# NoelShin/zutis

Measured on AMD Instinct MI355X. Metric: images/sec, COCO2017-val-shaped ViT-B/16 dense semantic segmentation @336px (ZUTIS forward + semantic predict), batches of 32 per GPU, 3 independent batches in flight, higher is better.
Workload: dtype f16x3 (fp32-class)

## Files before the change

### zutis_amd/csrc/attention.hip

```cpp
#include "common.h"
#include <type_traits>

struct AttnArgs {
  const half_t* Q; long ldq, sQ;
  const half_t* K; long ldk, sK;
  const half_t* V; long ldv, sV;
  half_t* O; long ldo, sO;
  int Tq, Tk, H, nqb, groups;
  float scale_log2;
  int causal;
  long planeQ, planeK, planeV, planeO;
  int ksplit, kchunk;
  float* part_o; float* part_m; float* part_l;
};

typedef __fp16 fp16x4 __attribute__((__vector_size__(4 * sizeof(__fp16))));
typedef __attribute__((address_space(3))) fp16x4* lds_fp16x4_ptr;

#define KT 64
#define VS 96

#define ZH_ATTN_LAZY_LOG2 8.0f

__device__ __forceinline__ float zh_xor32_max(float x) {
  float a = x, b = x;
  asm volatile("s_nop 1\n\tv_permlane32_swap_b32 %0, %1" : "+v"(a), "+v"(b));
  float r;
  asm("v_max_f32 %0, %1, %2" : "=v"(r) : "v"(a), "v"(b));
  return r;
}
__device__ __forceinline__ float zh_xor32_sum(float x) {
  float a = x, b = x;
  asm volatile("s_nop 1\n\tv_permlane32_swap_b32 %0, %1" : "+v"(a), "+v"(b));
  return a + b;
}

template <int DH, int NWAVE, int X3, int PIPE>
__global__ __launch_bounds__(64 * NWAVE, X3 ? 2 : (DH == 64 ? 3 : 2)) void attn_f16_kernel(AttnArgs p) {
  static_assert(!PIPE || X3, "the pipelined loop exists for the split-pair kernels");
  constexpr int NT = 64 * NWAVE;
  constexpr int KS = DH + 8;
  constexpr int NKS = DH / 16;
  constexpr int NDT = DH / 32;
  constexpr int CPR = DH / 8;
  constexpr int KTT = X3 ? 32 : KT;
  constexpr int NU = KTT / 32;
  constexpr int NLD = (KTT * CPR + NT - 1) / NT;
  constexpr bool LDFULL = (KTT * CPR) % NT == 0;
  __shared__ __attribute__((aligned(16))) half_t sKb[2][KTT * KS];
  __shared__ __attribute__((aligned(16))) half_t sKl[X3 ? 2 : 1][X3 ? KTT * KS : 8];
  __shared__ __attribute__((aligned(16))) half_t sVb[2][KTT * VS];
  __shared__ __attribute__((aligned(16))) half_t sVl[X3 ? 2 : 1][X3 ? KTT * VS : 8];

  const int tid = threadIdx.x, lane = tid & 63, wave = tid >> 6;
  const int id = blockIdx.y * gridDim.x + blockIdx.x;
  const int per_group = p.nqb * p.ksplit;
  const int item = (id & 7) * (int)(gridDim.x >> 3) + (id >> 3);
  if (item >= p.groups * per_group) return;
  const int group = item / per_group;
  const int qbs = item - group * per_group;
  const int qb = qbs / p.ksplit, ks = qbs - qb * p.ksplit;
  const int head = group % p.H, img = group / p.H;
  const int q0 = qb * (32 * NWAVE) + wave * 32;
  const int ql = lane & 31, hh = lane >> 5;
  const long hoff = (long)head * DH;

  const int key0 = ks * p.kchunk;
  const int key_end = p.ksplit > 1 ? min(p.Tk, key0 + p.kchunk) : p.Tk;
  const half_t* Q = p.Q + (long)img * p.sQ + hoff;
  const half_t* K = p.K + (long)img * p.sK + hoff;
  const half_t* V = p.V + (long)img * p.sV + hoff;

  half8_t qf[NKS], qfl[X3 ? NKS : 1];
  const half_t* qp = Q + (long)min(q0 + ql, p.Tq - 1) * p.ldq + 8 * hh;
#pragma unroll
  for (int ks = 0; ks < NKS; ++ks) qf[ks] = *(const half8_t*)(qp + 16 * ks);
  if (X3) {
#pragma unroll
    for (int ks = 0; ks < NKS; ++ks) qfl[ks] = *(const half8_t*)(qp + p.planeQ + 16 * ks);
  }

  f32x16 oacc[NDT];
#pragma unroll
  for (int d = 0; d < NDT; ++d)
#pragma unroll
    for (int r = 0; r < 16; ++r) oacc[d][r] = 0.f;
  float m_run = -INFINITY;
  f32x16 lacc;
#pragma unroll
  for (int r = 0; r < 16; ++r) lacc[r] = 0.f;
  float l_run = 0.f;
  half8_t ones;
#pragma unroll
  for (int i = 0; i < 8; ++i) ones[i] = (half_t)1.0f;

  struct TileRegs { half8_t k[NLD], v[NLD], kl[X3 ? NLD : 1], vl[X3 ? NLD : 1]; };
  TileRegs ra;
  const unsigned ldk2 = (unsigned)p.ldk * 2u, ldv2 = (unsigned)p.ldv * 2u;
  const char* const Kl = (const char*)(K + p.planeK);
  const char* const Vl = (const char*)(V + p.planeV);
  auto load_k = [&](int kbase, TileRegs& r) {
#pragma unroll
    for (int i = 0; i < NLD; ++i) {
      const int c = tid + i * NT;
      const int row = c / CPR, cc = c - row * CPR;
      if (LDFULL || c < KTT * CPR) {
        const unsigned ok = (unsigned)min(kbase + row, key_end - 1) * ldk2 + (unsigned)cc * 16u;
        r.k[i] = *(const half8_t*)((const char*)K + ok);
        if (X3) r.kl[i] = *(const half8_t*)(Kl + ok);
      }
    }
  };
  auto load_v = [&](int kbase, TileRegs& r) {
#pragma unroll
    for (int i = 0; i < NLD; ++i) {
      const int c = tid + i * NT;
      const int row = c / CPR, cc = c - row * CPR;
      if (LDFULL || c < KTT * CPR) {
        const unsigned ov = (unsigned)min(kbase + row, key_end - 1) * ldv2 + (unsigned)cc * 16u;
        r.v[i] = *(const half8_t*)((const char*)V + ov);
        if (X3) r.vl[i] = *(const half8_t*)(Vl + ov);
      }
    }
  };
  auto store_k = [&](int buf, const TileRegs& r) {
#pragma unroll
    for (int i = 0; i < NLD; ++i) {
      const int c = tid + i * NT;
      const int row = c / CPR, cc = c - row * CPR;
      if (LDFULL || c < KTT * CPR) {
        *(half8_t*)(sKb[buf] + row * KS + cc * 8) = r.k[i];
        if (X3) *(half8_t*)(sKl[buf] + row * KS + cc * 8) = r.kl[i];
      }
    }
  };
  auto store_v = [&](int buf, const TileRegs& r) {
#pragma unroll
    for (int i = 0; i < NLD; ++i) {
      const int c = tid + i * NT;
      const int row = c / CPR, cc = c - row * CPR;
      if (LDFULL || c < KTT * CPR) {
        *(half8_t*)(sVb[buf] + row * VS + cc * 8) = r.v[i];
        if (X3) *(half8_t*)(sVl[buf] + row * VS + cc * 8) = r.vl[i];
      }
    }
  };

  const int krow = (ql & 0x13) | ((ql & 4) << 1) | ((ql & 8) >> 1);
  const int tr_row = 8 * hh + ((lane & 15) >> 2);
  const int tr_col = 16 * ((lane >> 4) & 1) + 4 * (lane & 3);

  int ntiles = (max(key_end - key0, 0) + KTT - 1) / KTT;
  if (p.causal) {
    const int qlast = min(p.Tq, (qb + 1) * (32 * NWAVE)) - 1;
    ntiles = min(ntiles, qlast / KTT + 1);
  }
  const int qidx = q0 + ql;
  const bool active = q0 < p.Tq;

  auto qk = [&](int t, f32x16 (&s)[NU]) {
    const half_t* sK = sKb[t & 1];
#pragma unroll
    for (int u = 0; u < NU; ++u) {
#pragma unroll
      for (int r = 0; r < 16; ++r) s[u][r] = 0.f;
      const half_t* kp = sK + (32 * u + krow) * KS + 8 * hh;
#pragma unroll
      for (int ks = 0; ks < NKS; ++ks) {
        half8_t kf = *(const half8_t*)(kp + 16 * ks);
        half8_t kl;
        if (X3) kl = *(const half8_t*)(sKl[t & 1] + (32 * u + krow) * KS + 8 * hh + 16 * ks);
        s[u] = __builtin_amdgcn_mfma_f32_32x32x16_f16(kf, qf[ks], s[u], 0, 0, 0);
        if (X3) {
          s[u] = __builtin_amdgcn_mfma_f32_32x32x16_f16(kl, qf[ks], s[u], 0, 0, 0);
          s[u] = __builtin_amdgcn_mfma_f32_32x32x16_f16(kf, qfl[ks], s[u], 0, 0, 0);
        }
      }
    }
  };
  typedef unsigned u32x4 __attribute__((ext_vector_type(4)));
  struct PFrag { u32x4 hi[NU][2], lo[X3 ? NU : 1][2]; };
  auto softmax = [&](int t, f32x16 (&s)[NU], PFrag& P, auto masked) {
    constexpr bool MASKED = decltype(masked)::value;
    const int kbase = key0 + t * KTT;
    float mx = -INFINITY;
    if (MASKED && (kbase + KTT > key_end || (p.causal && kbase + KTT - 1 > q0))) {
#pragma unroll
      for (int u = 0; u < NU; ++u)
#pragma unroll
        for (int r = 0; r < 16; ++r) {
          const int key = kbase + 32 * u + 16 * (r >> 3) + 8 * hh + (r & 7);
          if (key >= key_end || (p.causal && key > qidx)) s[u][r] = -INFINITY;
        }
    }
    {
      float m4[4] = {mx, mx, mx, mx};
#pragma unroll
      for (int u = 0; u < NU; ++u)
#pragma unroll
        for (int r = 0; r < 16; r += 8) {
          m4[0] = fmaxf(fmaxf(m4[0], s[u][r + 0]), s[u][r + 1]);
          m4[1] = fmaxf(fmaxf(m4[1], s[u][r + 2]), s[u][r + 3]);
          m4[2] = fmaxf(fmaxf(m4[2], s[u][r + 4]), s[u][r + 5]);
          m4[3] = fmaxf(fmaxf(m4[3], s[u][r + 6]), s[u][r + 7]);
        }
      mx = fmaxf(fmaxf(m4[0], m4[1]), fmaxf(m4[2], m4[3]));
    }
    mx = zh_xor32_max(mx);
    const float m_cand = mx * p.scale_log2;
    const float m_new = m_cand > m_run + ZH_ATTN_LAZY_LOG2 ? m_cand : m_run;
    const float alpha = __builtin_amdgcn_exp2f(m_run - m_new);
    m_run = m_new;
    float lsum2[2] = {0.f, 0.f};
#pragma unroll
    for (int u = 0; u < NU; ++u)
#pragma unroll
      for (int r = 0; r < 16; r += 2) {
        const float e0 = __builtin_amdgcn_exp2f(__builtin_fmaf(s[u][r], p.scale_log2, -m_new));
        const float e1 = __builtin_amdgcn_exp2f(__builtin_fmaf(s[u][r + 1], p.scale_log2, -m_new));
        if (X3) { lsum2[0] += e0; lsum2[1] += e1; }
        const half2_t eh2 = {(half_t)e0, (half_t)e1};
        unsigned eh = __builtin_bit_cast(unsigned, eh2);
        if (X3) {
          unsigned el;
          asm("v_fma_mixlo_f16 %0, -%1, 1.0, %2 op_sel:[0,0,0] op_sel_hi:[1,0,0]\n\t"
              "v_fma_mixhi_f16 %0, -%1, 1.0, %3 op_sel:[1,0,0] op_sel_hi:[1,0,0]"
              : "=&v"(el) : "v"(eh), "v"(e0), "v"(e1));
          P.lo[u][r >> 3][(r >> 1) & 3] = el;
        }
        P.hi[u][r >> 3][(r >> 1) & 3] = eh;
      }
    if (__any(alpha != 1.0f)) {
#pragma unroll
      for (int d = 0; d < NDT; ++d)
#pragma unroll
        for (int r = 0; r < 16; ++r) oacc[d][r] *= alpha;
      if (!X3) {
#pragma unroll
        for (int r = 0; r < 16; ++r) lacc[r] *= alpha;
      }
    }
    if (X3) l_run = l_run * alpha + (lsum2[0] + lsum2[1]);
  };
  auto pv = [&](int t, const PFrag& P) {
    const half_t* sV = sVb[t & 1];
#pragma unroll
    for (int u = 0; u < NU; ++u)
#pragma unroll
      for (int ks = 0; ks < 2; ++ks) {
        if (!X3) lacc = __builtin_amdgcn_mfma_f32_32x32x16_f16(ones, __builtin_bit_cast(half8_t, P.hi[u][ks]), lacc, 0, 0, 0);
        const half_t* vp = sV + (32 * u + 16 * ks + tr_row) * VS + tr_col;
#pragma unroll
        for (int d = 0; d < NDT; ++d) {
          fp16x4 lo = __builtin_amdgcn_ds_read_tr16_b64_v4f16((lds_fp16x4_ptr)(vp + 32 * d));
          fp16x4 hi = __builtin_amdgcn_ds_read_tr16_b64_v4f16((lds_fp16x4_ptr)(vp + 32 * d + 4 * VS));
          half8_t vf;
          __builtin_memcpy(&vf, &lo, 8);
          __builtin_memcpy(((char*)&vf) + 8, &hi, 8);
          half8_t vl;
          if (X3) {
            const half_t* vq = sVl[t & 1] + (32 * u + 16 * ks + tr_row) * VS + tr_col;
            fp16x4 llo = __builtin_amdgcn_ds_read_tr16_b64_v4f16((lds_fp16x4_ptr)(vq + 32 * d));
            fp16x4 lhi = __builtin_amdgcn_ds_read_tr16_b64_v4f16((lds_fp16x4_ptr)(vq + 32 * d + 4 * VS));
            __builtin_memcpy(&vl, &llo, 8);
            __builtin_memcpy(((char*)&vl) + 8, &lhi, 8);
          }
          const half8_t pf = __builtin_bit_cast(half8_t, P.hi[u][ks]);
          oacc[d] = __builtin_amdgcn_mfma_f32_32x32x16_f16(vf, pf, oacc[d], 0, 0, 0);
          if (X3) {
            oacc[d] = __builtin_amdgcn_mfma_f32_32x32x16_f16(vl, pf, oacc[d], 0, 0, 0);
            oacc[d] = __builtin_amdgcn_mfma_f32_32x32x16_f16(vf, __builtin_bit_cast(half8_t, P.lo[u][ks]), oacc[d], 0, 0, 0);
          }
        }
      }
  };

  if (PIPE && !p.causal) {
    load_k(key0, ra);
    load_v(key0, ra);
    store_k(0, ra);
    store_v(0, ra);
    if (ntiles > 1) { load_k(key0 + KTT, ra); store_k(1, ra); }
    __syncthreads();
    f32x16 sA[NU], sB[NU];
    PFrag P;
    if (active) qk(0, sA);
    __syncthreads();
    auto step = [&](int t, auto par, f32x16 (&cur)[NU], f32x16 (&nxt)[NU]) {
      constexpr int PAR = decltype(par)::value;
      if (t + 2 < ntiles) load_k(key0 + (t + 2) * KTT, ra);
      load_v(key0 + (t + 1) * KTT, ra);
      if (active) {
        qk(PAR ^ 1, nxt);
        softmax(t, cur, P, std::false_type{});
        pv(PAR, P);
      }
      if (t + 2 < ntiles) store_k(PAR, ra);
      store_v(PAR ^ 1, ra);
      __syncthreads();
    };
    int t = 0;
    for (; t + 2 < ntiles; t += 2) {
      step(t, std::integral_constant<int, 0>{}, sA, sB);
      step(t + 1, std::integral_constant<int, 1>{}, sB, sA);
    }
    if (t + 1 < ntiles) {
      step(t, std::integral_constant<int, 0>{}, sA, sB);
      if (active) { softmax(t + 1, sB, P, std::true_type{}); pv(1, P); }
    } else if (active) {
      softmax(t, sA, P, std::true_type{});
      pv(0, P);
    }
  } else {
  auto load_tile = [&](int kbase, TileRegs& r) { load_k(kbase, r); load_v(kbase, r); };
  auto store_tile = [&](int buf, const TileRegs& r) { store_k(buf, r); store_v(buf, r); };
  load_tile(key0, ra);
  store_tile(0, ra);
  __syncthreads();
  auto compute = [&](int t) {
    if (active) {
      f32x16 s[NU];
      PFrag P;
      qk(t, s);
      softmax(t, s, P, std::true_type{});
      pv(t, P);
    }
  };

  for (int t = 0; t < ntiles; t += 2) {
    if (t + 1 < ntiles) load_tile(key0 + (t + 1) * KTT, ra);
    compute(t);
    if (t + 1 < ntiles) store_tile(1, ra);
    __syncthreads();
    if (t + 1 >= ntiles) break;
    if (t + 2 < ntiles) load_tile(key0 + (t + 2) * KTT, ra);
    compute(t + 1);
    if (t + 2 < ntiles) store_tile(0, ra);
    __syncthreads();
  }
  }

  for (int once = 0; once < 1; ++once) {
  const float l_row = X3 ? zh_xor32_sum(l_run) : lacc[0];
  const int qr = q0 + ql;
  if (p.ksplit > 1) {
    if (qr < p.Tq) {
      float* po = p.part_o + (((long)ks * (p.groups / p.H) + img) * p.Tq + qr) * ((long)p.H * DH) + hoff + 4 * hh;
#pragma unroll
      for (int d = 0; d < NDT; ++d)
#pragma unroll
        for (int g = 0; g < 4; ++g)
          *(f32x4*)(po + 32 * d + 8 * g) = (f32x4){oacc[d][4 * g], oacc[d][4 * g + 1], oacc[d][4 * g + 2], oacc[d][4 * g + 3]};
      if (hh == 0) {
        const long mi = ((long)ks * p.groups + group) * p.Tq + qr;
        p.part_m[mi] = m_run;
        p.part_l[mi] = l_row;
      }
    }
    continue;
  }
  const float inv = 1.0f / l_row;
  if (qr < p.Tq) {
    half_t* op = p.O + (long)img * p.sO + (long)qr * p.ldo + hoff + 4 * hh;
#pragma unroll
    for (int d = 0; d < NDT; ++d)
#pragma unroll
      for (int g = 0; g < 4; ++g) {
        const f32x4 o = {oacc[d][4 * g] * inv, oacc[d][4 * g + 1] * inv, oacc[d][4 * g + 2] * inv, oacc[d][4 * g + 3] * inv};
        zh_store_h4(op + 32 * d + 8 * g, p.planeO, o);
      }
  }
  }
}

__global__ __launch_bounds__(256) void attn_combine_kernel(const float* part_o, const float* part_m, const float* part_l, half_t* O, long ldo, long sO,
                                                           long planeO, int S, int B, int H, int Tq, int DH) {
  const int D = H * DH, c4 = D / 4;
  const long i = (long)blockIdx.x * 256 + threadIdx.x;
  if (i >= (long)B * Tq * c4) return;
  const int col = (int)(i % c4) * 4;
  const long row = i / c4;
  const int img = (int)(row / Tq), q = (int)(row - (long)img * Tq), head = col / DH;
  float m = -INFINITY;
  for (int s = 0; s < S; ++s) m = fmaxf(m, part_m[(((long)s * B + img) * H + head) * Tq + q]);
  f32x4 acc = {0.f, 0.f, 0.f, 0.f};
  float l = 0.f;
  for (int s = 0; s < S; ++s) {
    const long mi = (((long)s * B + img) * H + head) * Tq + q;
    const float w = __builtin_amdgcn_exp2f(part_m[mi] - m);
    l += w * part_l[mi];
    acc += *(const f32x4*)(part_o + (((long)s * B + img) * Tq + q) * D + col) * w;
  }
  const float inv = 1.0f / l;
  zh_store_h4(O + (long)img * sO + (long)q * ldo + col, planeO, acc * inv);
}

static int attention_launch(const void* Q, long ldq, long strideQ, const void* K, long ldk, long strideK,
                            const void* V, long ldv, long strideV, void* O, long ldo, long strideO,
                            int batch, int heads, int Tq, int Tk, int head_dim, float scale, int causal,
                            long planeQ, long planeK, long planeV, long planeO, hipStream_t stream, int ksplit = 1, void* workspace = nullptr,
                            size_t workspace_bytes = 0) {
  ZH_CHECK_ARG(Q && K && V && O, "zh_attention_f16: null operand");
  ZH_CHECK_ARG(batch > 0 && heads > 0 && Tq > 0 && Tk > 0, "zh_attention_f16: bad shape");
  ZH_CHECK_ARG(head_dim == 64 || head_dim == 96, "zh_attention_f16: head_dim %d not in {64, 96}", head_dim);
  ZH_CHECK_ARG(ldq % 8 == 0 && ldk % 8 == 0 && ldv % 8 == 0 && ldo % 4 == 0 && strideQ % 8 == 0 && strideK % 8 == 0 &&
                   strideV % 8 == 0 && strideO % 4 == 0 && planeQ % 8 == 0 && planeK % 8 == 0 && planeV % 8 == 0 && planeO % 4 == 0,
               "zh_attention_f16: row/batch/plane strides must keep 16-byte (Q,K,V) / 8-byte (O) alignment");
  ZH_CHECK_ARG(((uintptr_t)Q & 15) == 0 && ((uintptr_t)K & 15) == 0 && ((uintptr_t)V & 15) == 0 && ((uintptr_t)O & 7) == 0,
               "zh_attention_f16: misaligned pointer");
  ZH_CHECK_ARG(heads < 65536 && batch < 65536, "zh_attention_f16: heads/batch exceed grid limits");
  ZH_CHECK_ARG((long)Tk * ldk * 2 < (1L << 32) && (long)Tk * ldv * 2 < (1L << 32), "zh_attention_f16: Tk * ldk (ldv) exceeds 2^31 elements");
  ZH_CHECK_ARG((planeQ != 0) == (planeK != 0) && (planeQ != 0) == (planeV != 0),
               "zh_attention_f16: the split-pair mode needs the lo planes of Q, K and V (all three or none)");
  AttnArgs p;
  p.Q = (const half_t*)Q; p.ldq = ldq; p.sQ = strideQ;
  p.K = (const half_t*)K; p.ldk = ldk; p.sK = strideK;
  p.V = (const half_t*)V; p.ldv = ldv; p.sV = strideV;
  p.O = (half_t*)O; p.ldo = ldo; p.sO = strideO;
  p.Tq = Tq; p.Tk = Tk; p.H = heads;
  p.scale_log2 = scale * 1.4426950408889634f;
  p.causal = causal;
  p.planeQ = planeQ; p.planeK = planeK; p.planeV = planeV; p.planeO = planeO;
  const bool x3 = planeQ != 0;
  p.nqb = zh_cdiv(Tq, 128);
  p.groups = heads * batch;
  p.ksplit = 1; p.kchunk = 0; p.part_o = p.part_m = p.part_l = nullptr;
  if (ksplit > 1) {
    ZH_CHECK_ARG(!causal && ksplit <= 64, "zh_attention_f16_splitk: ksplit %d not in 1..64 (and not for the causal form)", ksplit);
    const int ktt = x3 ? 32 : 64;
    p.ksplit = ksplit;
    p.kchunk = zh_cdiv(zh_cdiv(Tk, ktt), ksplit) * ktt;
    ZH_CHECK_ARG((long)(ksplit - 1) * p.kchunk < Tk, "zh_attention_f16_splitk: ksplit %d leaves an empty key chunk for Tk = %d", ksplit, Tk);
    const size_t no = (size_t)ksplit * batch * Tq * heads * head_dim, nm = (size_t)ksplit * batch * heads * Tq;
    ZH_CHECK_ARG(workspace && workspace_bytes >= (no + 2 * nm) * 4 && ((uintptr_t)workspace & 15) == 0,
                 "zh_attention_f16_splitk: workspace too small or misaligned (%zu < %zu)", workspace_bytes, (no + 2 * nm) * 4);
    p.part_o = (float*)workspace; p.part_m = p.part_o + no; p.part_l = p.part_m + nm;
  }
  const long items = (long)p.groups * p.nqb * p.ksplit;
  ZH_CHECK_ARG(items < (1L << 31) - 8, "zh_attention_f16: grid too large");
  const long nblk = (long)zh_cdiv(items, 8) * 8;
  ZH_CHECK_ARG(nblk < (1L << 31), "zh_attention_f16: grid too large");
  dim3 grid((unsigned)nblk);
  const bool pipe = x3 && (head_dim == 96 || zh_cdiv(nblk, 512L) <= zh_cdiv(nblk, 768L));
  if (head_dim == 64) {
    if (x3 && pipe) hipLaunchKernelGGL((attn_f16_kernel<64, 4, 1, 1>), grid, dim3(256), 0, stream, p);
    else if (x3) hipLaunchKernelGGL((attn_f16_kernel<64, 4, 1, 0>), grid, dim3(256), 0, stream, p);
    else hipLaunchKernelGGL((attn_f16_kernel<64, 4, 0, 0>), grid, dim3(256), 0, stream, p);
  } else {
    if (x3 && pipe) hipLaunchKernelGGL((attn_f16_kernel<96, 4, 1, 1>), grid, dim3(256), 0, stream, p);
    else if (x3) hipLaunchKernelGGL((attn_f16_kernel<96, 4, 1, 0>), grid, dim3(256), 0, stream, p);
    else hipLaunchKernelGGL((attn_f16_kernel<96, 4, 0, 0>), grid, dim3(256), 0, stream, p);
  }
  ZH_CHECK_LAUNCH("zh_attention_f16");
  if (p.ksplit > 1) {
    const long n4 = (long)batch * Tq * heads * head_dim / 4;
    hipLaunchKernelGGL(attn_combine_kernel, dim3((unsigned)zh_cdiv(n4, 256)), dim3(256), 0, stream, p.part_o, p.part_m, p.part_l, p.O, ldo, strideO,
                       planeO, p.ksplit, batch, heads, Tq, head_dim);
    ZH_CHECK_LAUNCH("zh_attention_f16_splitk (combine)");
  }
  return ZH_OK;
}

extern "C" size_t zh_attention_splitk_workspace_size(int batch, int heads, int Tq, int head_dim, int ksplit) {
  return ((size_t)ksplit * batch * Tq * heads * head_dim + 2 * (size_t)ksplit * batch * heads * Tq) * 4;
}
extern "C" int zh_attention_f16_splitk(const void* Q, long ldq, long strideQ, const void* K, long ldk, long strideK,
                                       const void* V, long ldv, long strideV, void* O, long ldo, long strideO,
                                       int batch, int heads, int Tq, int Tk, int head_dim, float scale,
                                       long planeQ, long planeK, long planeV, long planeO, int ksplit, void* workspace, size_t workspace_bytes,
                                       hipStream_t stream) {
  return attention_launch(Q, ldq, strideQ, K, ldk, strideK, V, ldv, strideV, O, ldo, strideO, batch, heads, Tq, Tk, head_dim,
                          scale, 0, planeQ, planeK, planeV, planeO, stream, ksplit, workspace, workspace_bytes);
}

extern "C" int zh_attention_f16(const void* Q, long ldq, long strideQ, const void* K, long ldk, long strideK,
                                const void* V, long ldv, long strideV, void* O, long ldo, long strideO,
                                int batch, int heads, int Tq, int Tk, int head_dim, float scale,
                                long planeQ, long planeK, long planeV, long planeO, hipStream_t stream) {
  return attention_launch(Q, ldq, strideQ, K, ldk, strideK, V, ldv, strideV, O, ldo, strideO, batch, heads, Tq, Tk, head_dim,
                          scale, 0, planeQ, planeK, planeV, planeO, stream);
}

extern "C" int zh_attention_causal_f16(const void* Q, long ldq, long strideQ, const void* K, long ldk, long strideK,
                                       const void* V, long ldv, long strideV, void* O, long ldo, long strideO,
                                       int batch, int heads, int T, int head_dim, float scale,
                                       long planeQ, long planeK, long planeV, long planeO, hipStream_t stream) {
  return attention_launch(Q, ldq, strideQ, K, ldk, strideK, V, ldv, strideV, O, ldo, strideO, batch, heads, T, T, head_dim,
                          scale, 1, planeQ, planeK, planeV, planeO, stream);
}
```

Before: 3073.

## Stream K/V tiles into LDS via direct global-to-LDS DMA with 3-stage ring

For the split-pair (X3) attention kernels, K and V tiles are now loaded straight from global memory into LDS with global_load_lds_dwordx4 instead of going through registers and ds_write. A three-stage ring buffer with vmcnt-based partial waits replaces the old register double-buffering. The LDS layout becomes unpadded and XOR-swizzled, and the qk and pv read addressing is changed to match. This is meant to free VGPRs and the issue slots spent on LDS stores, and to hide more load latency. The cost is extra LDS per block, reliance on hand-written inline asm for m0 and waitcnt, and tricky counter bookkeeping that can cause races if it is wrong.

```diff
diff --git a/zutis_amd/csrc/attention.hip b/zutis_amd/csrc/attention.hip
--- a/zutis_amd/csrc/attention.hip
+++ b/zutis_amd/csrc/attention.hip
@@ -18,7 +18,6 @@
 typedef __attribute__((address_space(3))) fp16x4* lds_fp16x4_ptr;
 
 #define KT 64
-#define VS 96
 
 #define ZH_ATTN_LAZY_LOG2 8.0f
 
@@ -35,22 +34,49 @@
   return a + b;
 }
 
+__device__ __forceinline__ void attn_dma16(unsigned lds, unsigned off, const char* base) {
+  asm volatile("s_nop 2\n\ts_mov_b32 m0, %0\n\ts_nop 0\n\tglobal_load_lds_dwordx4 %1, %2" :: "s"(lds), "v"(off), "s"(base) : "memory");
+}
+__device__ __forceinline__ const char* attn_sgpr_ptr(const void* ptr) {
+  const uintptr_t v = (uintptr_t)ptr;
+  return (const char*)(((uintptr_t)(unsigned)__builtin_amdgcn_readfirstlane((int)(v >> 32)) << 32) |
+                       (uintptr_t)(unsigned)__builtin_amdgcn_readfirstlane((int)(unsigned)v));
+}
+template <int NP, int MAXC>
+__device__ __forceinline__ void attn_wait_barrier(int c) {
+  static_assert(MAXC * NP < 64, "vmcnt is a 6-bit counter");
+  if constexpr (MAXC > 0) {
+    if (c >= MAXC) {
+      asm volatile("s_waitcnt vmcnt(%0) lgkmcnt(0)\n\ts_barrier" :: "n"(MAXC * NP) : "memory");
+      return;
+    }
+    attn_wait_barrier<NP, MAXC - 1>(c);
+  } else {
+    asm volatile("s_waitcnt vmcnt(0) lgkmcnt(0)\n\ts_barrier" ::: "memory");
+  }
+}
+
 template <int DH, int NWAVE, int X3, int PIPE>
 __global__ __launch_bounds__(64 * NWAVE, X3 ? 2 : (DH == 64 ? 3 : 2)) void attn_f16_kernel(AttnArgs p) {
   static_assert(!PIPE || X3, "the pipelined loop exists for the split-pair kernels");
-  constexpr int NT = 64 * NWAVE;
-  constexpr int KS = DH + 8;
   constexpr int NKS = DH / 16;
   constexpr int NDT = DH / 32;
   constexpr int CPR = DH / 8;
   constexpr int KTT = X3 ? 32 : KT;
   constexpr int NU = KTT / 32;
+  constexpr int PLANE = KTT * DH;
+  constexpr int STAGE = 4 * PLANE;
+  constexpr int NST = 3;
+  constexpr int PPP = PLANE / 512;
+  constexpr int NPW = 2 * PPP / NWAVE;
+  static_assert(!X3 || 2 * PPP % NWAVE == 0, "whole pieces per wave");
+  constexpr int KS = DH + 8, VS = 96;
+  constexpr int NT = 64 * NWAVE;
   constexpr int NLD = (KTT * CPR + NT - 1) / NT;
   constexpr bool LDFULL = (KTT * CPR) % NT == 0;
-  __shared__ __attribute__((aligned(16))) half_t sKb[2][KTT * KS];
-  __shared__ __attribute__((aligned(16))) half_t sKl[X3 ? 2 : 1][X3 ? KTT * KS : 8];
-  __shared__ __attribute__((aligned(16))) half_t sVb[2][KTT * VS];
-  __shared__ __attribute__((aligned(16))) half_t sVl[X3 ? 2 : 1][X3 ? KTT * VS : 8];
+  __shared__ __attribute__((aligned(16))) half_t smem[X3 ? NST * STAGE : 2 * KTT * (KS + VS)];
+  auto k_at = [&](int st) { return smem + (X3 ? st * STAGE : st * KTT * KS); };
+  auto v_at = [&](int st) { return smem + (X3 ? st * STAGE + 2 * PLANE : 2 * KTT * KS + st * KTT * VS); };
 
   const int tid = threadIdx.x, lane = tid & 63, wave = tid >> 6;
   const int id = blockIdx.y * gridDim.x + blockIdx.x;
@@ -71,85 +97,6 @@
   const half_t* K = p.K + (long)img * p.sK + hoff;
   const half_t* V = p.V + (long)img * p.sV + hoff;
 
-  half8_t qf[NKS], qfl[X3 ? NKS : 1];
-  const half_t* qp = Q + (long)min(q0 + ql, p.Tq - 1) * p.ldq + 8 * hh;
-#pragma unroll
-  for (int ks = 0; ks < NKS; ++ks) qf[ks] = *(const half8_t*)(qp + 16 * ks);
-  if (X3) {
-#pragma unroll
-    for (int ks = 0; ks < NKS; ++ks) qfl[ks] = *(const half8_t*)(qp + p.planeQ + 16 * ks);
-  }
-
-  f32x16 oacc[NDT];
-#pragma unroll
-  for (int d = 0; d < NDT; ++d)
-#pragma unroll
-    for (int r = 0; r < 16; ++r) oacc[d][r] = 0.f;
-  float m_run = -INFINITY;
-  f32x16 lacc;
-#pragma unroll
-  for (int r = 0; r < 16; ++r) lacc[r] = 0.f;
-  float l_run = 0.f;
-  half8_t ones;
-#pragma unroll
-  for (int i = 0; i < 8; ++i) ones[i] = (half_t)1.0f;
-
-  struct TileRegs { half8_t k[NLD], v[NLD], kl[X3 ? NLD : 1], vl[X3 ? NLD : 1]; };
-  TileRegs ra;
-  const unsigned ldk2 = (unsigned)p.ldk * 2u, ldv2 = (unsigned)p.ldv * 2u;
-  const char* const Kl = (const char*)(K + p.planeK);
-  const char* const Vl = (const char*)(V + p.planeV);
-  auto load_k = [&](int kbase, TileRegs& r) {
-#pragma unroll
-    for (int i = 0; i < NLD; ++i) {
-      const int c = tid + i * NT;
-      const int row = c / CPR, cc = c - row * CPR;
-      if (LDFULL || c < KTT * CPR) {
-        const unsigned ok = (unsigned)min(kbase + row, key_end - 1) * ldk2 + (unsigned)cc * 16u;
-        r.k[i] = *(const half8_t*)((const char*)K + ok);
-        if (X3) r.kl[i] = *(const half8_t*)(Kl + ok);
-      }
-    }
-  };
-  auto load_v = [&](int kbase, TileRegs& r) {
-#pragma unroll
-    for (int i = 0; i < NLD; ++i) {
-      const int c = tid + i * NT;
-      const int row = c / CPR, cc = c - row * CPR;
-      if (LDFULL || c < KTT * CPR) {
-        const unsigned ov = (unsigned)min(kbase + row, key_end - 1) * ldv2 + (unsigned)cc * 16u;
-        r.v[i] = *(const half8_t*)((const char*)V + ov);
-        if (X3) r.vl[i] = *(const half8_t*)(Vl + ov);
-      }
-    }
-  };
-  auto store_k = [&](int buf, const TileRegs& r) {
-#pragma unroll
-    for (int i = 0; i < NLD; ++i) {
-      const int c = tid + i * NT;
-      const int row = c / CPR, cc = c - row * CPR;
-      if (LDFULL || c < KTT * CPR) {
-        *(half8_t*)(sKb[buf] + row * KS + cc * 8) = r.k[i];
-        if (X3) *(half8_t*)(sKl[buf] + row * KS + cc * 8) = r.kl[i];
-      }
-    }
-  };
-  auto store_v = [&](int buf, const TileRegs& r) {
-#pragma unroll
-    for (int i = 0; i < NLD; ++i) {
-      const int c = tid + i * NT;
-      const int row = c / CPR, cc = c - row * CPR;
-      if (LDFULL || c < KTT * CPR) {
-        *(half8_t*)(sVb[buf] + row * VS + cc * 8) = r.v[i];
-        if (X3) *(half8_t*)(sVl[buf] + row * VS + cc * 8) = r.vl[i];
-      }
-    }
-  };
-
-  const int krow = (ql & 0x13) | ((ql & 4) << 1) | ((ql & 8) >> 1);
-  const int tr_row = 8 * hh + ((lane & 15) >> 2);
-  const int tr_col = 16 * ((lane >> 4) & 1) + 4 * (lane & 3);
-
   int ntiles = (max(key_end - key0, 0) + KTT - 1) / KTT;
   if (p.causal) {
     const int qlast = min(p.Tq, (qb + 1) * (32 * NWAVE)) - 1;
@@ -158,18 +105,126 @@
   const int qidx = q0 + ql;
   const bool active = q0 < p.Tq;
 
-  auto qk = [&](int t, f32x16 (&s)[NU]) {
-    const half_t* sK = sKb[t & 1];
+  const int wv = __builtin_amdgcn_readfirstlane(wave);
+  const unsigned ldk2 = (unsigned)p.ldk * 2u, ldv2 = (unsigned)p.ldv * 2u;
+  const char* ksrc[X3 ? NPW : 1];
+  const char* vsrc[X3 ? NPW : 1];
+  unsigned plds[X3 ? NPW : 1], pkc[X3 ? NPW : 1], pvc[X3 ? NPW : 1];
+  int prow[X3 ? NPW : 1];
+#pragma unroll
+  for (int i = 0; i < (X3 ? NPW : 0); ++i) {
+    const int q = wv + NWAVE * i;
+    const int pl = PPP % NWAVE == 0 ? NWAVE * i / PPP : q / PPP;
+    const int j = q - pl * PPP;
+    const int c = 64 * j + lane;
+    const int blk = c / (8 * CPR), w8 = c - blk * (8 * CPR);
+    const int r = 8 * blk + ((w8 >> 2) & 7), ch = 4 * (w8 >> 5) + (w8 & 3);
+    prow[i] = r;
+    pkc[i] = (unsigned)(ch ^ ((r >> 2) & 3)) * 16u;
+    pvc[i] = (unsigned)ch * 16u;
+    plds[i] = (unsigned)(pl * PLANE * 2 + j * 1024);
+    ksrc[i] = attn_sgpr_ptr(K + pl * p.planeK);
+    vsrc[i] = attn_sgpr_ptr(V + pl * p.planeV);
+  }
+  const unsigned lds0 = (unsigned)(uintptr_t)smem;
+  auto key_row = [&](int t, int i) { return (unsigned)min(key0 + t * KTT + prow[i], key_end - 1); };
+  auto dma_k = [&](int t, int st) {
+#pragma unroll
+    for (int i = 0; i < NPW; ++i) attn_dma16(lds0 + (unsigned)(st * STAGE * 2) + plds[i], key_row(t, i) * ldk2 + pkc[i], ksrc[i]);
+  };
+  auto dma_v = [&](int t, int st) {
+#pragma unroll
+    for (int i = 0; i < NPW; ++i)
+      attn_dma16(lds0 + (unsigned)((st * STAGE + 2 * PLANE) * 2) + plds[i], key_row(t, i) * ldv2 + pvc[i], vsrc[i]);
+  };
+  half8_t rk[X3 ? 1 : NLD], rv[X3 ? 1 : NLD];
+  auto load_tile = [&](int t) {
+#pragma unroll
+    for (int i = 0; i < (X3 ? 0 : NLD); ++i) {
+      const int c = tid + i * NT;
+      const int row = c / CPR, cc = c - row * CPR;
+      if (LDFULL || c < KTT * CPR) rk[i] = *(const half8_t*)((const char*)K + ((unsigned)min(key0 + t * KTT + row, key_end - 1) * ldk2 + (unsigned)cc * 16u));
+    }
+#pragma unroll
+    for (int i = 0; i < (X3 ? 0 : NLD); ++i) {
+      const int c = tid + i * NT;
+      const int row = c / CPR, cc = c - row * CPR;
+      if (LDFULL || c < KTT * CPR) rv[i] = *(const half8_t*)((const char*)V + ((unsigned)min(key0 + t * KTT + row, key_end - 1) * ldv2 + (unsigned)cc * 16u));
+    }
+  };
+  auto store_tile = [&](int st) {
+#pragma unroll
+    for (int i = 0; i < (X3 ? 0 : NLD); ++i) {
+      const int c = tid + i * NT;
+      const int row = c / CPR, cc = c - row * CPR;
+      if (LDFULL || c < KTT * CPR) *(half8_t*)(k_at(st) + row * KS + cc * 8) = rk[i];
+    }
+#pragma unroll
+    for (int i = 0; i < (X3 ? 0 : NLD); ++i) {
+      const int c = tid + i * NT;
+      const int row = c / CPR, cc = c - row * CPR;
+      if (LDFULL || c < KTT * CPR) *(half8_t*)(v_at(st) + row * VS + cc * 8) = rv[i];
+    }
+  };
+
+  const bool piped = PIPE && !p.causal;
+  if constexpr (X3) {
+    if (piped) {
+      dma_k(0, 0);
+#pragma unroll
+      for (int s = 1; s < NST; ++s) {
+        if (s < ntiles) dma_k(s, s);
+        if (s - 1 < ntiles) dma_v(s - 1, s - 1);
+      }
+    } else {
+#pragma unroll
+      for (int s = 0; s + 1 < NST; ++s)
+        if (s < ntiles) { dma_k(s, s); dma_v(s, s); }
+    }
+  }
+
+  half8_t qf[NKS], qfl[X3 ? NKS : 1];
+  const half_t* qp = Q + (long)min(q0 + ql, p.Tq - 1) * p.ldq + 8 * hh;
+#pragma unroll
+  for (int ks = 0; ks < NKS; ++ks) qf[ks] = *(const half8_t*)(qp + 16 * ks);
+  if (X3) {
+#pragma unroll
+    for (int ks = 0; ks < NKS; ++ks) qfl[ks] = *(const half8_t*)(qp + p.planeQ + 16 * ks);
+  }
+  if constexpr (X3) __builtin_amdgcn_s_waitcnt(0x0F70);
+
+  f32x16 oacc[NDT];
+#pragma unroll
+  for (int d = 0; d < NDT; ++d)
+#pragma unroll
+    for (int r = 0; r < 16; ++r) oacc[d][r] = 0.f;
+  float m_run = -INFINITY;
+  f32x16 lacc;
+#pragma unroll
+  for (int r = 0; r < 16; ++r) lacc[r] = 0.f;
+  float l_run = 0.f;
+  half8_t ones;
+#pragma unroll
+  for (int i = 0; i < 8; ++i) ones[i] = (half_t)1.0f;
+
+  const int krow = (ql & 0x13) | ((ql & 4) << 1) | ((ql & 8) >> 1);
+  const int kre = 8 * ((krow >> 3) * 8 * CPR + (krow & 7) * 4 + (hh ^ ((krow >> 2) & 3)));
+  const int kro = kre ^ 16;
+  const int vrd = X3 ? 8 * (hh * 8 * CPR + ((lane >> 2) & 3) * 4 + 2 * ((lane >> 4) & 1) + ((lane >> 1) & 1)) + 4 * (lane & 1)
+                     : (8 * hh + ((lane & 15) >> 2)) * VS + 16 * ((lane >> 4) & 1) + 4 * (lane & 3);
+
+  auto qk = [&](int st, f32x16 (&s)[NU]) {
+    const half_t* sK = k_at(st);
 #pragma unroll
     for (int u = 0; u < NU; ++u) {
 #pragma unroll
       for (int r = 0; r < 16; ++r) s[u][r] = 0.f;
-      const half_t* kp = sK + (32 * u + krow) * KS + 8 * hh;
 #pragma unroll
       for (int ks = 0; ks < NKS; ++ks) {
-        half8_t kf = *(const half8_t*)(kp + 16 * ks);
+        const half_t* kp = X3 ? sK + ((ks & 1) ? kro : kre) + 32 * DH * u + 256 * (ks >> 1) : sK + (32 * u + krow) * KS + 8 * hh + 16 * ks;
+        half8_t kf = *(const half8_t*)kp;
         half8_t kl;
-        if (X3) kl = *(const half8_t*)(sKl[t & 1] + (32 * u + krow) * KS + 8 * hh + 16 * ks);
+        if (X3) kl = *(const half8_t*)(kp + PLANE);
         s[u] = __builtin_amdgcn_mfma_f32_32x32x16_f16(kf, qf[ks], s[u], 0, 0, 0);
         if (X3) {
           s[u] = __builtin_amdgcn_mfma_f32_32x32x16_f16(kl, qf[ks], s[u], 0, 0, 0);
@@ -242,26 +297,26 @@
     }
     if (X3) l_run = l_run * alpha + (lsum2[0] + lsum2[1]);
   };
-  auto pv = [&](int t, const PFrag& P) {
-    const half_t* sV = sVb[t & 1];
+  auto pv = [&](int st, const PFrag& P) {
+    const half_t* sV = v_at(st);
+    constexpr int DV = X3 ? 256 : 32, RV = X3 ? 128 : 4 * VS;
 #pragma unroll
     for (int u = 0; u < NU; ++u)
 #pragma unroll
       for (int ks = 0; ks < 2; ++ks) {
         if (!X3) lacc = __builtin_amdgcn_mfma_f32_32x32x16_f16(ones, __builtin_bit_cast(half8_t, P.hi[u][ks]), lacc, 0, 0, 0);
-        const half_t* vp = sV + (32 * u + 16 * ks + tr_row) * VS + tr_col;
+        const half_t* vp = sV + vrd + (X3 ? 32 * DH * u + 16 * DH * ks : (32 * u + 16 * ks) * VS);
 #pragma unroll
         for (int d = 0; d < NDT; ++d) {
-          fp16x4 lo = __builtin_amdgcn_ds_read_tr16_b64_v4f16((lds_fp16x4_ptr)(vp + 32 * d));
-          fp16x4 hi = __builtin_amdgcn_ds_read_tr16_b64_v4f16((lds_fp16x4_ptr)(vp + 32 * d + 4 * VS));
+          fp16x4 lo = __builtin_amdgcn_ds_read_tr16_b64_v4f16((lds_fp16x4_ptr)(vp + DV * d));
+          fp16x4 hi = __builtin_amdgcn_ds_read_tr16_b64_v4f16((lds_fp16x4_ptr)(vp + DV * d + RV));
           half8_t vf;
           __builtin_memcpy(&vf, &lo, 8);
           __builtin_memcpy(((char*)&vf) + 8, &hi, 8);
           half8_t vl;
           if (X3) {
-            const half_t* vq = sVl[t & 1] + (32 * u + 16 * ks + tr_row) * VS + tr_col;
-            fp16x4 llo = __builtin_amdgcn_ds_read_tr16_b64_v4f16((lds_fp16x4_ptr)(vq + 32 * d));
-            fp16x4 lhi = __builtin_amdgcn_ds_read_tr16_b64_v4f16((lds_fp16x4_ptr)(vq + 32 * d + 4 * VS));
+            fp16x4 llo = __builtin_amdgcn_ds_read_tr16_b64_v4f16((lds_fp16x4_ptr)(vp + PLANE + DV * d));
+            fp16x4 lhi = __builtin_amdgcn_ds_read_tr16_b64_v4f16((lds_fp16x4_ptr)(vp + PLANE + DV * d + RV));
             __builtin_memcpy(&vl, &llo, 8);
             __builtin_memcpy(((char*)&vl) + 8, &lhi, 8);
           }
@@ -275,69 +330,77 @@
       }
   };
 
-  if (PIPE && !p.causal) {
-    load_k(key0, ra);
-    load_v(key0, ra);
-    store_k(0, ra);
-    store_v(0, ra);
-    if (ntiles > 1) { load_k(key0 + KTT, ra); store_k(1, ra); }
+  if constexpr (X3) {
+    if (piped) {
+      attn_wait_barrier<1, 0>(0);
+      f32x16 sA[NU], sB[NU];
+      PFrag P;
+      if (active) qk(0, sA);
+      attn_wait_barrier<1, 0>(0);
+      auto step = [&](int t, f32x16 (&cur)[NU], f32x16 (&nxt)[NU]) {
+        if (t + NST < ntiles) dma_k(t + NST, t % NST);
+        if (t + NST - 1 < ntiles) dma_v(t + NST - 1, (t + NST - 1) % NST);
+        if (active) {
+          qk((t + 1) % NST, nxt);
+          softmax(t, cur, P, std::false_type{});
+          pv(t % NST, P);
+        }
+        const int nk = max(min(t + NST, ntiles - 1) - max(t + 3, NST) + 1, 0);
+        const int nv = max(min(t + NST - 1, ntiles - 1) - max(t + 2, NST - 1) + 1, 0);
+        attn_wait_barrier<NPW, 2 * (NST - 2)>(nk + nv);
+      };
+      int t = 0;
+      for (; t + 2 < ntiles; t += 2) {
+        step(t, sA, sB);
+        step(t + 1, sB, sA);
+      }
+      if (t + 1 < ntiles) {
+        step(t, sA, sB);
+        if (active) { softmax(t + 1, sB, P, std::true_type{}); pv((t + 1) % NST, P); }
+      } else if (active) {
+        softmax(t, sA, P, std::true_type{});
+        pv(t % NST, P);
+      }
+    } else {
+      for (int t = 0; t < ntiles; ++t) {
+        attn_wait_barrier<2 * NPW, NST - 2>(max(min(t + NST - 2, ntiles - 1) - max(t + 1, NST - 1) + 1, 0));
+        if (t + NST - 1 < ntiles) {
+          dma_k(t + NST - 1, (t + NST - 1) % NST);
+          dma_v(t + NST - 1, (t + NST - 1) % NST);
+        }
+        if (active) {
+          f32x16 s[NU];
+          PFrag P;
+          qk(t % NST, s);
+          softmax(t, s, P, std::true_type{});
+          pv(t % NST, P);
+        }
+      }
+    }
+  } else {
+    load_tile(0);
+    store_tile(0);
     __syncthreads();
-    f32x16 sA[NU], sB[NU];
-    PFrag P;
-    if (active) qk(0, sA);
-    __syncthreads();
-    auto step = [&](int t, auto par, f32x16 (&cur)[NU], f32x16 (&nxt)[NU]) {
-      constexpr int PAR = decltype(par)::value;
-      if (t + 2 < ntiles) load_k(key0 + (t + 2) * KTT, ra);
-      load_v(key0 + (t + 1) * KTT, ra);
+    auto compute = [&](int t, int st) {
       if (active) {
-        qk(PAR ^ 1, nxt);
-        softmax(t, cur, P, std::false_type{});
-        pv(PAR, P);
-      }
-      if (t + 2 < ntiles) store_k(PAR, ra);
-      store_v(PAR ^ 1, ra);
+        f32x16 s[NU];
+        PFrag P;
+        qk(st, s);
+        softmax(t, s, P, std::true_type{});
+        pv(st, P);
+      }
+    };
+    for (int t = 0; t < ntiles; t += 2) {
+      if (t + 1 < ntiles) load_tile(t + 1);
+      compute(t, 0);
+      if (t + 1 < ntiles) store_tile(1);
       __syncthreads();
-    };
-    int t = 0;
-    for (; t + 2 < ntiles; t += 2) {
-      step(t, std::integral_constant<int, 0>{}, sA, sB);
-      step(t + 1, std::integral_constant<int, 1>{}, sB, sA);
-    }
-    if (t + 1 < ntiles) {
-      step(t, std::integral_constant<int, 0>{}, sA, sB);
-      if (active) { softmax(t + 1, sB, P, std::true_type{}); pv(1, P); }
-    } else if (active) {
-      softmax(t, sA, P, std::true_type{});
-      pv(0, P);
-    }
-  } else {
-  auto load_tile = [&](int kbase, TileRegs& r) { load_k(kbase, r); load_v(kbase, r); };
-  auto store_tile = [&](int buf, const TileRegs& r) { store_k(buf, r); store_v(buf, r); };
-  load_tile(key0, ra);
-  store_tile(0, ra);
-  __syncthreads();
-  auto compute = [&](int t) {
-    if (active) {
-      f32x16 s[NU];
-      PFrag P;
-      qk(t, s);
-      softmax(t, s, P, std::true_type{});
-      pv(t, P);
-    }
-  };
-
-  for (int t = 0; t < ntiles; t += 2) {
-    if (t + 1 < ntiles) load_tile(key0 + (t + 1) * KTT, ra);
-    compute(t);
-    if (t + 1 < ntiles) store_tile(1, ra);
-    __syncthreads();
-    if (t + 1 >= ntiles) break;
-    if (t + 2 < ntiles) load_tile(key0 + (t + 2) * KTT, ra);
-    compute(t + 1);
-    if (t + 2 < ntiles) store_tile(0, ra);
-    __syncthreads();
-  }
+      if (t + 1 >= ntiles) break;
+      if (t + 2 < ntiles) load_tile(t + 2);
+      compute(t + 1, 1);
+      if (t + 2 < ntiles) store_tile(0);
+      __syncthreads();
+    }
   }
 
   for (int once = 0; once < 1; ++once) {
```

Result: no change. 3082 (median of 6 runs) (+0.3%).
